# raulmur/ORB_SLAM2

Hardware: NVIDIA H100
Metric: stereo frames/sec (ORB extract L+R + ComputeStereoMatches, KITTI-shaped 1242x375 @2000 kpts) (higher is better)
Workload: dtype u8

## Files before the change

orb_slam2_b200/csrc/k_quadtree.cu:

```cuda
#include "borb_internal.h"

namespace borb {

namespace {

typedef unsigned long long u64;

struct QtView {
    short *bx0[2], *bx1[2], *by0[2], *by1[2];
    int* cnt[2];
    int *cc, *tbl, *order, *scanA, *scanB, *divided, *misc;
    u64* keys;
};

__host__ __device__ inline int pow2_ge(int v) { int k = 1; while (k < v) k <<= 1; return k; }

__device__ inline QtView carve(unsigned char* base, int C, int K) {
    QtView v;
    u64* k = reinterpret_cast<u64*>(base);
    v.keys = k;
    int* ip = reinterpret_cast<int*>(k + K);
    v.cnt[0] = ip; ip += C;
    v.cnt[1] = ip; ip += C;
    v.cc = ip; ip += 4 * C;
    v.tbl = ip; ip += 4 * C;
    v.order = ip; ip += C;
    v.scanA = ip; ip += C;
    v.scanB = ip; ip += C;
    v.divided = ip; ip += C;
    v.misc = ip; ip += 40;
    short* sp = reinterpret_cast<short*>(ip);
    for (int b = 0; b < 2; b++) {
        v.bx0[b] = sp; sp += C;
        v.bx1[b] = sp; sp += C;
        v.by0[b] = sp; sp += C;
        v.by1[b] = sp; sp += C;
    }
    return v;
}

__device__ int block_exscan(int* a, int m, int* wsum) {
    const int T = blockDim.x, tid = threadIdx.x, lane = tid & 31, w = tid >> 5, nw = T >> 5;
    const int per = (m + T - 1) / T;
    const int beg = min(tid * per, m), end = min(beg + per, m);
    int s = 0;
    for (int i = beg; i < end; i++) s += a[i];
    int incl = s;
#pragma unroll
    for (int off = 1; off < 32; off <<= 1) {
        int t = __shfl_up_sync(0xFFFFFFFFu, incl, off);
        if (lane >= off) incl += t;
    }
    if (lane == 31) wsum[w] = incl;
    __syncthreads();
    if (w == 0) {
        int v = lane < nw ? wsum[lane] : 0;
        int inc2 = v;
#pragma unroll
        for (int off = 1; off < 32; off <<= 1) {
            int t = __shfl_up_sync(0xFFFFFFFFu, inc2, off);
            if (lane >= off) inc2 += t;
        }
        wsum[lane] = inc2 - v;
        if (lane == 31) wsum[32] = inc2;
    }
    __syncthreads();
    int base = wsum[w] + incl - s;
    const int total = wsum[32];
    for (int i = beg; i < end; i++) {
        int t = a[i];
        a[i] = base;
        base += t;
    }
    __syncthreads();
    return total;
}

__device__ __forceinline__ int quadrant(int x, int y, int x0, int x1, int y0, int y1) {
    const int mx = x0 + ((x1 - x0 + 1) >> 1);
    const int my = y0 + ((y1 - y0 + 1) >> 1);
    return (x < mx) ? ((y < my) ? 0 : 2) : ((y < my) ? 1 : 3);
}

}

size_t quadtree_smem_bytes(int node_cap) {
    const int C = node_cap, K = pow2_ge(C);
    return (size_t)K * 8 + (size_t)(2 * C + 8 * C + 4 * C) * 4 + 40 * 4 + (size_t)8 * C * 2 + 64;
}

__global__ void __launch_bounds__(256) quadtree_kernel(const __grid_constant__ Geometry g, const uint32_t* __restrict__ cand,
                                                       const int* __restrict__ cand_cnt, int* __restrict__ pnode,
                                                       uint32_t* __restrict__ sel, int* __restrict__ sel_cnt) {
    extern __shared__ __align__(16) unsigned char smem_raw[];
    const int img = blockIdx.y, l = blockIdx.x;
    const LevelGeom& L = g.lv[l];
    const int tid = threadIdx.x, T = blockDim.x;
    const int C = L.node_cap, K = pow2_ge(C);
    QtView v = carve(smem_raw, C, K);
    const int P = min(cand_cnt[img * g.nlevels + l], L.cand_cap);
    const int N = L.quota;
    const uint32_t* pts = cand + (size_t)img * g.cand_image_stride + L.cand_off;
    int* pn = pnode + (size_t)img * g.cand_image_stride + L.cand_off;
    uint32_t* out = sel + (size_t)img * g.sel_image_stride + L.sel_off;
    if (P == 0) {
        if (tid == 0) sel_cnt[img * g.nlevels + l] = 0;
        return;
    }
    const int nIni = L.nIni;
    const float hX = L.hX;
    for (int i = tid; i < nIni; i += T) v.cc[i] = 0;
    __syncthreads();
    for (int p = tid; p < P; p += T) {
        const int x = xys_x(pts[p]) - MIN_BORDER;
        int r = (int)__fdiv_rn((float)x, hX);
        r = min(max(r, 0), nIni - 1);
        atomicAdd(&v.cc[r], 1);
        pn[p] = r;
    }
    __syncthreads();
    for (int i = tid; i < nIni; i += T) v.scanA[i] = v.cc[i] > 0;
    __syncthreads();
    int n = block_exscan(v.scanA, nIni, v.misc);
    int cur = 0;
    for (int i = tid; i < nIni; i += T)
        if (v.cc[i] > 0) {
            const int j = v.scanA[i];
            v.bx0[0][j] = (short)(int)__fmul_rn(hX, (float)i);
            v.bx1[0][j] = (short)(int)__fmul_rn(hX, (float)(i + 1));
            v.by0[0][j] = 0;
            v.by1[0][j] = (short)(L.h - 2 * MIN_BORDER);
            v.cnt[0][j] = v.cc[i];
            v.tbl[i] = j;
        }
    __syncthreads();
    for (int p = tid; p < P; p += T) pn[p] = v.tbl[pn[p]];
    __syncthreads();

    bool phase2 = false, finish = false;
    while (!finish) {
        const int prevSize = n;
        const short *X0 = v.bx0[cur], *X1 = v.bx1[cur], *Y0 = v.by0[cur], *Y1 = v.by1[cur];
        const int* CN = v.cnt[cur];
        for (int j = tid; j < 4 * n; j += T) v.cc[j] = 0;
        __syncthreads();
        for (int p = tid; p < P; p += T) {
            const int k = pn[p];
            if (CN[k] > 1) {
                const uint32_t e = pts[p];
                const int q = quadrant(xys_x(e) - MIN_BORDER, xys_y(e) - MIN_BORDER, X0[k], X1[k], Y0[k], Y1[k]);
                atomicAdd(&v.cc[4 * k + q], 1);
            }
        }
        __syncthreads();
        for (int k = tid; k < n; k += T) v.scanA[k] = CN[k] > 1;
        __syncthreads();
        const int E = block_exscan(v.scanA, n, v.misc);
        int Dn = E;
        if (!phase2) {
            for (int k = tid; k < n; k += T)
                if (CN[k] > 1) v.order[v.scanA[k]] = k;
            __syncthreads();
        } else {
            for (int i = tid; i < K; i += T)
                v.keys[i] = (i < n && CN[i] > 1) ? (((u64)(0xFFFFFFFFu - (unsigned)CN[i]) << 32) | (unsigned)i) : ~0ull;
            __syncthreads();
            for (int kk = 2; kk <= K; kk <<= 1)
                for (int j = kk >> 1; j > 0; j >>= 1) {
                    for (int i = tid; i < K; i += T) {
                        const int ixj = i ^ j;
                        if (ixj > i) {
                            const bool asc = (i & kk) == 0;
                            const u64 a = v.keys[i], b = v.keys[ixj];
                            if ((a > b) == asc) { v.keys[i] = b; v.keys[ixj] = a; }
                        }
                    }
                    __syncthreads();
                }
            for (int r = tid; r < E; r += T) v.order[r] = (int)(v.keys[r] & 0xFFFFFFFFull);
            if (tid == 0) v.misc[33] = E;
            __syncthreads();
            for (int r = tid; r < E; r += T) {
                const int k = v.order[r];
                v.scanA[r] = (v.cc[4 * k] > 0) + (v.cc[4 * k + 1] > 0) + (v.cc[4 * k + 2] > 0) + (v.cc[4 * k + 3] > 0) - 1;
            }
            __syncthreads();
            block_exscan(v.scanA, E, v.misc);
            for (int r = tid; r < E; r += T) {
                const int k = v.order[r];
                const int d = (v.cc[4 * k] > 0) + (v.cc[4 * k + 1] > 0) + (v.cc[4 * k + 2] > 0) + (v.cc[4 * k + 3] > 0) - 1;
                if (n + v.scanA[r] + d >= N) atomicMin(&v.misc[33], r);
            }
            __syncthreads();
            Dn = min(v.misc[33] + 1, E);
            __syncthreads();
        }
        for (int k = tid; k < n; k += T) v.divided[k] = 0;
        __syncthreads();
        for (int r = tid; r < Dn; r += T) v.divided[v.order[r]] = 1;
        for (int r = tid; r < E; r += T) {
            const int k = v.order[r];
            v.scanA[r] = r < Dn ? (v.cc[4 * k] > 0) + (v.cc[4 * k + 1] > 0) + (v.cc[4 * k + 2] > 0) + (v.cc[4 * k + 3] > 0) : 0;
        }
        __syncthreads();
        const int totalCreated = block_exscan(v.scanA, E, v.misc);
        for (int k = tid; k < n; k += T) v.scanB[k] = !v.divided[k];
        __syncthreads();
        const int totalUnd = block_exscan(v.scanB, n, v.misc);
        const int nxt = cur ^ 1;
        if (tid == 0) v.misc[34] = 0;
        __syncthreads();
        int big = 0;
        for (int r = tid; r < Dn; r += T) {
            const int k = v.order[r];
            int c = v.scanA[r];
            const int x0 = X0[k], x1 = X1[k], y0 = Y0[k], y1 = Y1[k];
            const int mx = x0 + ((x1 - x0 + 1) >> 1), my = y0 + ((y1 - y0 + 1) >> 1);
#pragma unroll
            for (int q = 0; q < 4; q++) {
                const int cq = v.cc[4 * k + q];
                if (cq > 0) {
                    const int j = totalCreated - 1 - c;
                    c++;
                    v.tbl[4 * k + q] = j;
                    v.bx0[nxt][j] = (short)((q & 1) ? mx : x0);
                    v.bx1[nxt][j] = (short)((q & 1) ? x1 : mx);
                    v.by0[nxt][j] = (short)((q & 2) ? my : y0);
                    v.by1[nxt][j] = (short)((q & 2) ? y1 : my);
                    v.cnt[nxt][j] = cq;
                    big += cq > 1;
                }
            }
        }
        for (int k = tid; k < n; k += T)
            if (!v.divided[k]) {
                const int j = totalCreated + v.scanB[k];
                v.tbl[4 * k] = j;
                v.bx0[nxt][j] = X0[k]; v.bx1[nxt][j] = X1[k]; v.by0[nxt][j] = Y0[k]; v.by1[nxt][j] = Y1[k];
                v.cnt[nxt][j] = CN[k];
            }
        if (big) atomicAdd(&v.misc[34], big);
        __syncthreads();
        for (int p = tid; p < P; p += T) {
            const int k = pn[p];
            if (v.divided[k]) {
                const uint32_t e = pts[p];
                const int q = quadrant(xys_x(e) - MIN_BORDER, xys_y(e) - MIN_BORDER, X0[k], X1[k], Y0[k], Y1[k]);
                pn[p] = v.tbl[4 * k + q];
            } else
                pn[p] = v.tbl[4 * k];
        }
        const int nToExpand = v.misc[34];
        n = totalCreated + totalUnd;
        cur = nxt;
        __syncthreads();
        if (n >= N || n == prevSize) finish = true;
        else if (!phase2 && n + 3 * nToExpand > N) phase2 = true;
    }
    u64* best = v.keys;
    for (int k = tid; k < n; k += T) best[k] = 0;
    __syncthreads();
    const u64 ORD_MASK = (1ull << 40) - 1;
    for (int p = tid; p < P; p += T) {
        const uint32_t e = pts[p];
        const int x = xys_x(e), y = xys_y(e);
        const u64 ord = ((u64)((y - EDGE) / L.hCell) << 32) | ((u64)((x - EDGE) / L.wCell) << 24) | ((u64)y << 12) | (u64)x;
        const u64 key = ((u64)xys_s(e) << 40) | (ORD_MASK - ord);
        atomicMax(&best[pn[p]], key);
    }
    __syncthreads();
    for (int k = tid; k < n; k += T) {
        const u64 key = best[k];
        const u64 ord = ORD_MASK - (key & ORD_MASK);
        out[k] = pack_xys((int)(ord & 0xFFF), (int)((ord >> 12) & 0xFFF), (int)(key >> 40));
    }
    if (tid == 0) sel_cnt[img * g.nlevels + l] = n;
}

int launch_quadtree(const Geometry& g, const Workspace& ws, int n_images, cudaStream_t s) {
    int maxC = 0;
    for (int l = 0; l < g.nlevels; l++) maxC = g.lv[l].node_cap > maxC ? g.lv[l].node_cap : maxC;
    const size_t smem = quadtree_smem_bytes(maxC);
    allow_max_smem((const void*)quadtree_kernel);
    dim3 grid(g.nlevels, n_images);
    quadtree_kernel<<<grid, 256, smem, s>>>(g, ws.cand, ws.cand_cnt, ws.pnode, ws.sel, ws.sel_cnt);
    return 1;
}

}
```

Before: 37720.

## Restructure quadtree kernel: register-resident points, fused scans, rank-based ordering

Rewrites the ORB quadtree distribution kernel. Candidate points and their node ids are held in registers when the count fits (up to 20 per thread), so per-iteration global reads and writes of pnode are avoided. Node boxes are packed as short4. Divide and keep are fused into a single scan callback with a packed 16/16-bit counter, and the next level's vote is done right after the move, removing several passes and barriers. The phase-2 bitonic sort is replaced with an O(n^2) rank count, which is cheaper for small node counts but scales poorly if nodes grow, and the extra registers may cost occupancy.

```diff
diff --git a/orb_slam2_b200/csrc/k_quadtree.cu b/orb_slam2_b200/csrc/k_quadtree.cu
--- a/orb_slam2_b200/csrc/k_quadtree.cu
+++ b/orb_slam2_b200/csrc/k_quadtree.cu
@@ -4,47 +4,47 @@
 
 namespace {
 
-typedef unsigned long long u64;
+constexpr int QT_THREADS = 256;
+constexpr int QT_PPT = 20;
+constexpr int QT_ONCHIP = QT_THREADS * QT_PPT;
 
 struct QtView {
-    short *bx0[2], *bx1[2], *by0[2], *by1[2];
+    int* cc[2];
+    short4* box[2];
     int* cnt[2];
-    int *cc, *tbl, *order, *scanA, *scanB, *divided, *misc;
-    u64* keys;
+    int* tbl;
+    int* order;
+    int* rank;
+    int* pre;
+    int* misc;
 };
 
-__host__ __device__ inline int pow2_ge(int v) { int k = 1; while (k < v) k <<= 1; return k; }
-
-__device__ inline QtView carve(unsigned char* base, int C, int K) {
+__device__ inline QtView carve(unsigned char* base, int C) {
     QtView v;
-    u64* k = reinterpret_cast<u64*>(base);
-    v.keys = k;
-    int* ip = reinterpret_cast<int*>(k + K);
+    int* ip = reinterpret_cast<int*>(base);
+    v.cc[0] = ip; ip += 4 * C;
+    v.cc[1] = ip; ip += 4 * C;
+    short4* bp = reinterpret_cast<short4*>(ip);
+    v.box[0] = bp; bp += C;
+    v.box[1] = bp; bp += C;
+    ip = reinterpret_cast<int*>(bp);
     v.cnt[0] = ip; ip += C;
     v.cnt[1] = ip; ip += C;
-    v.cc = ip; ip += 4 * C;
     v.tbl = ip; ip += 4 * C;
     v.order = ip; ip += C;
-    v.scanA = ip; ip += C;
-    v.scanB = ip; ip += C;
-    v.divided = ip; ip += C;
-    v.misc = ip; ip += 40;
-    short* sp = reinterpret_cast<short*>(ip);
-    for (int b = 0; b < 2; b++) {
-        v.bx0[b] = sp; sp += C;
-        v.bx1[b] = sp; sp += C;
-        v.by0[b] = sp; sp += C;
-        v.by1[b] = sp; sp += C;
-    }
+    v.rank = ip; ip += C;
+    v.pre = ip; ip += C + 1;
+    v.misc = ip;
     return v;
 }
 
-__device__ int block_exscan(int* a, int m, int* wsum) {
-    const int T = blockDim.x, tid = threadIdx.x, lane = tid & 31, w = tid >> 5, nw = T >> 5;
-    const int per = (m + T - 1) / T;
+template <class V, class U>
+__device__ __forceinline__ int block_exscan(int m, int* wsum, V val, U use) {
+    const int tid = threadIdx.x, lane = tid & 31, w = tid >> 5, nw = QT_THREADS >> 5;
+    const int per = (m + QT_THREADS - 1) / QT_THREADS;
     const int beg = min(tid * per, m), end = min(beg + per, m);
     int s = 0;
-    for (int i = beg; i < end; i++) s += a[i];
+    for (int i = beg; i < end; i++) s += val(i);
     int incl = s;
 #pragma unroll
     for (int off = 1; off < 32; off <<= 1) {
@@ -54,50 +54,70 @@
     if (lane == 31) wsum[w] = incl;
     __syncthreads();
     if (w == 0) {
-        int v = lane < nw ? wsum[lane] : 0;
-        int inc2 = v;
+        int x = lane < nw ? wsum[lane] : 0;
+        int inc2 = x;
 #pragma unroll
         for (int off = 1; off < 32; off <<= 1) {
             int t = __shfl_up_sync(0xFFFFFFFFu, inc2, off);
             if (lane >= off) inc2 += t;
         }
-        wsum[lane] = inc2 - v;
+        wsum[lane] = inc2 - x;
         if (lane == 31) wsum[32] = inc2;
     }
     __syncthreads();
     int base = wsum[w] + incl - s;
     const int total = wsum[32];
     for (int i = beg; i < end; i++) {
-        int t = a[i];
-        a[i] = base;
+        const int t = val(i);
+        use(i, base, total);
         base += t;
     }
-    __syncthreads();
     return total;
 }
 
-__device__ __forceinline__ int quadrant(int x, int y, int x0, int x1, int y0, int y1) {
-    const int mx = x0 + ((x1 - x0 + 1) >> 1);
-    const int my = y0 + ((y1 - y0 + 1) >> 1);
+__device__ __forceinline__ int quadrant(uint32_t e, short4 b) {
+    const int x = xys_x(e) - MIN_BORDER, y = xys_y(e) - MIN_BORDER;
+    const int mx = b.x + ((b.y - b.x + 1) >> 1);
+    const int my = b.z + ((b.w - b.z + 1) >> 1);
     return (x < mx) ? ((y < my) ? 0 : 2) : ((y < my) ? 1 : 3);
 }
 
+template <bool READ, bool WRITE, class F>
+__device__ __forceinline__ void for_points(bool onchip, int P, const uint32_t (&e)[QT_PPT], uint32_t (&nd)[QT_PPT / 2],
+                                           const uint32_t* __restrict__ pts, int* __restrict__ pn, F f) {
+    if (onchip) {
+#pragma unroll
+        for (int i = 0; i < QT_PPT; i++)
+            if (threadIdx.x + i * QT_THREADS < P) {
+                const int sh = 16 * (i & 1);
+                int s = (nd[i / 2] >> sh) & 0xFFFF;
+                f(e[i], s);
+                if (WRITE) nd[i / 2] = (nd[i / 2] & ~(0xFFFFu << sh)) | ((uint32_t)s << sh);
+            }
+    } else {
+        for (int p = threadIdx.x; p < P; p += QT_THREADS) {
+            int s = READ ? pn[p] : 0;
+            f(pts[p], s);
+            if (WRITE) pn[p] = s;
+        }
+    }
+}
+
 }
 
 size_t quadtree_smem_bytes(int node_cap) {
-    const int C = node_cap, K = pow2_ge(C);
-    return (size_t)K * 8 + (size_t)(2 * C + 8 * C + 4 * C) * 4 + 40 * 4 + (size_t)8 * C * 2 + 64;
-}
-
-__global__ void __launch_bounds__(256) quadtree_kernel(const __grid_constant__ Geometry g, const uint32_t* __restrict__ cand,
-                                                       const int* __restrict__ cand_cnt, int* __restrict__ pnode,
-                                                       uint32_t* __restrict__ sel, int* __restrict__ sel_cnt) {
+    const size_t C = (size_t)node_cap;
+    return C * (2 * 4 * 4 + 2 * 8 + 2 * 4 + 4 * 4 + 3 * 4) + 4 + 35 * 4;
+}
+
+__global__ void __launch_bounds__(QT_THREADS, 4) quadtree_kernel(const __grid_constant__ Geometry g, const uint32_t* __restrict__ cand,
+                                                                 const int* __restrict__ cand_cnt, int* __restrict__ pnode,
+                                                                 uint32_t* __restrict__ sel, int* __restrict__ sel_cnt) {
     extern __shared__ __align__(16) unsigned char smem_raw[];
     const int img = blockIdx.y, l = blockIdx.x;
     const LevelGeom& L = g.lv[l];
-    const int tid = threadIdx.x, T = blockDim.x;
-    const int C = L.node_cap, K = pow2_ge(C);
-    QtView v = carve(smem_raw, C, K);
+    const int tid = threadIdx.x, T = QT_THREADS;
+    QtView v = carve(smem_raw, L.node_cap);
     const int P = min(cand_cnt[img * g.nlevels + l], L.cand_cap);
     const int N = L.quota;
     const uint32_t* pts = cand + (size_t)img * g.cand_image_stride + L.cand_off;
@@ -107,174 +127,141 @@
         if (tid == 0) sel_cnt[img * g.nlevels + l] = 0;
         return;
     }
+    const bool onchip = P <= QT_ONCHIP;
+    uint32_t e[QT_PPT], nd[QT_PPT / 2] = {};
+    if (onchip) {
+#pragma unroll
+        for (int i = 0; i < QT_PPT; i++) e[i] = tid + i * T < P ? pts[tid + i * T] : 0u;
+    }
     const int nIni = L.nIni;
     const float hX = L.hX;
-    for (int i = tid; i < nIni; i += T) v.cc[i] = 0;
-    __syncthreads();
-    for (int p = tid; p < P; p += T) {
-        const int x = xys_x(pts[p]) - MIN_BORDER;
-        int r = (int)__fdiv_rn((float)x, hX);
-        r = min(max(r, 0), nIni - 1);
-        atomicAdd(&v.cc[r], 1);
-        pn[p] = r;
-    }
-    __syncthreads();
-    for (int i = tid; i < nIni; i += T) v.scanA[i] = v.cc[i] > 0;
-    __syncthreads();
-    int n = block_exscan(v.scanA, nIni, v.misc);
-    int cur = 0;
-    for (int i = tid; i < nIni; i += T)
-        if (v.cc[i] > 0) {
-            const int j = v.scanA[i];
-            v.bx0[0][j] = (short)(int)__fmul_rn(hX, (float)i);
-            v.bx1[0][j] = (short)(int)__fmul_rn(hX, (float)(i + 1));
-            v.by0[0][j] = 0;
-            v.by1[0][j] = (short)(L.h - 2 * MIN_BORDER);
-            v.cnt[0][j] = v.cc[i];
+    int* rc = v.cc[1];
+    for (int i = tid; i < nIni; i += T) rc[i] = 0;
+    __syncthreads();
+    for_points<false, true>(onchip, P, e, nd, pts, pn, [&](uint32_t x, int& s) {
+        const int r = (int)__fdiv_rn((float)(xys_x(x) - MIN_BORDER), hX);
+        s = min(max(r, 0), nIni - 1);
+        atomicAdd(&rc[s], 1);
+    });
+    __syncthreads();
+    int n = block_exscan(nIni, v.misc, [&](int i) { return rc[i] > 0; }, [&](int i, int j, int) {
+        if (rc[i] > 0) {
+            v.box[0][j] = make_short4((short)(int)__fmul_rn(hX, (float)i), (short)(int)__fmul_rn(hX, (float)(i + 1)), 0,
+                                      (short)(L.h - 2 * MIN_BORDER));
+            v.cnt[0][j] = rc[i];
             v.tbl[i] = j;
         }
-    __syncthreads();
-    for (int p = tid; p < P; p += T) pn[p] = v.tbl[pn[p]];
-    __syncthreads();
-
-    bool phase2 = false, finish = false;
-    while (!finish) {
-        const int prevSize = n;
-        const short *X0 = v.bx0[cur], *X1 = v.bx1[cur], *Y0 = v.by0[cur], *Y1 = v.by1[cur];
-        const int* CN = v.cnt[cur];
-        for (int j = tid; j < 4 * n; j += T) v.cc[j] = 0;
-        __syncthreads();
-        for (int p = tid; p < P; p += T) {
-            const int k = pn[p];
-            if (CN[k] > 1) {
-                const uint32_t e = pts[p];
-                const int q = quadrant(xys_x(e) - MIN_BORDER, xys_y(e) - MIN_BORDER, X0[k], X1[k], Y0[k], Y1[k]);
-                atomicAdd(&v.cc[4 * k + q], 1);
-            }
-        }
-        __syncthreads();
-        for (int k = tid; k < n; k += T) v.scanA[k] = CN[k] > 1;
-        __syncthreads();
-        const int E = block_exscan(v.scanA, n, v.misc);
-        int Dn = E;
-        if (!phase2) {
-            for (int k = tid; k < n; k += T)
-                if (CN[k] > 1) v.order[v.scanA[k]] = k;
-            __syncthreads();
-        } else {
-            for (int i = tid; i < K; i += T)
-                v.keys[i] = (i < n && CN[i] > 1) ? (((u64)(0xFFFFFFFFu - (unsigned)CN[i]) << 32) | (unsigned)i) : ~0ull;
-            __syncthreads();
-            for (int kk = 2; kk <= K; kk <<= 1)
-                for (int j = kk >> 1; j > 0; j >>= 1) {
-                    for (int i = tid; i < K; i += T) {
-                        const int ixj = i ^ j;
-                        if (ixj > i) {
-                            const bool asc = (i & kk) == 0;
-                            const u64 a = v.keys[i], b = v.keys[ixj];
-                            if ((a > b) == asc) { v.keys[i] = b; v.keys[ixj] = a; }
-                        }
-                    }
-                    __syncthreads();
-                }
-            for (int r = tid; r < E; r += T) v.order[r] = (int)(v.keys[r] & 0xFFFFFFFFull);
-            if (tid == 0) v.misc[33] = E;
-            __syncthreads();
-            for (int r = tid; r < E; r += T) {
-                const int k = v.order[r];
-                v.scanA[r] = (v.cc[4 * k] > 0) + (v.cc[4 * k + 1] > 0) + (v.cc[4 * k + 2] > 0) + (v.cc[4 * k + 3] > 0) - 1;
-            }
-            __syncthreads();
-            block_exscan(v.scanA, E, v.misc);
-            for (int r = tid; r < E; r += T) {
-                const int k = v.order[r];
-                const int d = (v.cc[4 * k] > 0) + (v.cc[4 * k + 1] > 0) + (v.cc[4 * k + 2] > 0) + (v.cc[4 * k + 3] > 0) - 1;
-                if (n + v.scanA[r] + d >= N) atomicMin(&v.misc[33], r);
-            }
-            __syncthreads();
-            Dn = min(v.misc[33] + 1, E);
-            __syncthreads();
-        }
-        for (int k = tid; k < n; k += T) v.divided[k] = 0;
-        __syncthreads();
-        for (int r = tid; r < Dn; r += T) v.divided[v.order[r]] = 1;
-        for (int r = tid; r < E; r += T) {
-            const int k = v.order[r];
-            v.scanA[r] = r < Dn ? (v.cc[4 * k] > 0) + (v.cc[4 * k + 1] > 0) + (v.cc[4 * k + 2] > 0) + (v.cc[4 * k + 3] > 0) : 0;
-        }
-        __syncthreads();
-        const int totalCreated = block_exscan(v.scanA, E, v.misc);
-        for (int k = tid; k < n; k += T) v.scanB[k] = !v.divided[k];
-        __syncthreads();
-        const int totalUnd = block_exscan(v.scanB, n, v.misc);
-        const int nxt = cur ^ 1;
-        if (tid == 0) v.misc[34] = 0;
-        __syncthreads();
+    });
+    for (int j = n + tid; j < ((n + 3) & ~3); j += T) v.cnt[0][j] = 0;
+    for (int j = tid; j < 4 * n; j += T) v.cc[0][j] = 0;
+    __syncthreads();
+    short4 *B = v.box[0], *NB = v.box[1];
+    int *CN = v.cnt[0], *NCN = v.cnt[1], *CC = v.cc[0], *NCC = v.cc[1];
+    auto move_and_vote = [&](const short4* bx, int* cc) {
+        for_points<true, true>(onchip, P, e, nd, pts, pn, [&](uint32_t x, int& s) {
+            const int k = v.tbl[s];
+            s = 4 * k + quadrant(x, bx[k]);
+        });
+        for_points<true, false>(onchip, P, e, nd, pts, pn, [&](uint32_t, int& s) { atomicAdd(&cc[s], 1); });
+    };
+    move_and_vote(B, CC);
+    __syncthreads();
+
+    int E = 0, nn;
+    bool phase2 = false;
+    for (;;) {
+        auto children = [&](int k) { return (CC[4 * k] > 0) + (CC[4 * k + 1] > 0) + (CC[4 * k + 2] > 0) + (CC[4 * k + 3] > 0); };
         int big = 0;
-        for (int r = tid; r < Dn; r += T) {
-            const int k = v.order[r];
-            int c = v.scanA[r];
-            const int x0 = X0[k], x1 = X1[k], y0 = Y0[k], y1 = Y1[k];
-            const int mx = x0 + ((x1 - x0 + 1) >> 1), my = y0 + ((y1 - y0 + 1) >> 1);
+        auto divide = [&](int k, int j) {
+            const short4 b = B[k];
+            const short mx = (short)(b.x + ((b.y - b.x + 1) >> 1)), my = (short)(b.z + ((b.w - b.z + 1) >> 1));
 #pragma unroll
             for (int q = 0; q < 4; q++) {
-                const int cq = v.cc[4 * k + q];
+                const int cq = CC[4 * k + q];
                 if (cq > 0) {
-                    const int j = totalCreated - 1 - c;
-                    c++;
                     v.tbl[4 * k + q] = j;
-                    v.bx0[nxt][j] = (short)((q & 1) ? mx : x0);
-                    v.bx1[nxt][j] = (short)((q & 1) ? x1 : mx);
-                    v.by0[nxt][j] = (short)((q & 2) ? my : y0);
-                    v.by1[nxt][j] = (short)((q & 2) ? y1 : my);
-                    v.cnt[nxt][j] = cq;
+                    NB[j] = make_short4((q & 1) ? mx : b.x, (q & 1) ? b.y : mx, (q & 2) ? my : b.z, (q & 2) ? b.w : my);
+                    NCN[j] = cq;
                     big += cq > 1;
+                    j--;
                 }
             }
-        }
-        for (int k = tid; k < n; k += T)
-            if (!v.divided[k]) {
-                const int j = totalCreated + v.scanB[k];
-                v.tbl[4 * k] = j;
-                v.bx0[nxt][j] = X0[k]; v.bx1[nxt][j] = X1[k]; v.by0[nxt][j] = Y0[k]; v.by1[nxt][j] = Y1[k];
-                v.cnt[nxt][j] = CN[k];
+        };
+        auto keep = [&](int k, int j) {
+            v.tbl[4 * k] = v.tbl[4 * k + 1] = v.tbl[4 * k + 2] = v.tbl[4 * k + 3] = j;
+            NB[j] = B[k];
+            NCN[j] = CN[k];
+        };
+        if (tid == 0) v.misc[34] = 0;
+        int created;
+        if (!phase2) {
+            const int tot = block_exscan(n, v.misc, [&](int k) { return CN[k] > 1 ? children(k) << 16 : 1; }, [&](int k, int pre, int total) {
+                if (CN[k] > 1) divide(k, (total >> 16) - 1 - (pre >> 16));
+                else keep(k, (total >> 16) + (pre & 0xFFFF));
+            });
+            created = tot >> 16;
+            nn = created + (tot & 0xFFFF);
+        } else {
+            const int4* CN4 = reinterpret_cast<const int4*>(CN);
+            for (int k = tid; k < n; k += T) {
+                const int s = CN[k];
+                if (s > 1) {
+                    int r = 0;
+                    for (int j = 0; j < n; j += 4) {
+                        const int4 c = CN4[j >> 2];
+                        r += (c.x + (j < k) > s) + (c.y + (j + 1 < k) > s) + (c.z + (j + 2 < k) > s) + (c.w + (j + 3 < k) > s);
+                    }
+                    v.order[r] = k;
+                    v.rank[k] = r;
+                } else
+                    v.rank[k] = E;
             }
+            if (tid == 0) { v.misc[33] = E; v.pre[0] = 0; }
+            __syncthreads();
+            block_exscan(E, v.misc, [&](int r) { return children(v.order[r]) - 1; }, [&](int r, int pre, int) {
+                const int d = children(v.order[r]) - 1;
+                v.pre[r + 1] = pre + d;
+                if (n + pre + d >= N) atomicMin(&v.misc[33], r);
+            });
+            __syncthreads();
+            const int Dn = min(v.misc[33] + 1, E);
+            created = v.pre[Dn] + Dn;
+            for (int r = tid; r < Dn; r += T) divide(v.order[r], created - 1 - v.pre[r] - r);
+            nn = created + block_exscan(n, v.misc, [&](int k) { return v.rank[k] >= Dn; }, [&](int k, int pre, int) {
+                if (v.rank[k] >= Dn) keep(k, created + pre);
+            });
+        }
         if (big) atomicAdd(&v.misc[34], big);
+        const bool last = nn >= N || nn == n;
+        for (int j = tid; j < 4 * nn; j += T) NCC[j] = 0;
+        for (int j = nn + tid; j < ((nn + 3) & ~3); j += T) NCN[j] = 0;
         __syncthreads();
-        for (int p = tid; p < P; p += T) {
-            const int k = pn[p];
-            if (v.divided[k]) {
-                const uint32_t e = pts[p];
-                const int q = quadrant(xys_x(e) - MIN_BORDER, xys_y(e) - MIN_BORDER, X0[k], X1[k], Y0[k], Y1[k]);
-                pn[p] = v.tbl[4 * k + q];
-            } else
-                pn[p] = v.tbl[4 * k];
-        }
+        if (last) break;
         const int nToExpand = v.misc[34];
-        n = totalCreated + totalUnd;
-        cur = nxt;
+        move_and_vote(NB, NCC);
         __syncthreads();
-        if (n >= N || n == prevSize) finish = true;
-        else if (!phase2 && n + 3 * nToExpand > N) phase2 = true;
-    }
-    u64* best = v.keys;
-    for (int k = tid; k < n; k += T) best[k] = 0;
-    __syncthreads();
+        if (!phase2 && nn + 3 * nToExpand > N) phase2 = true;
+        n = nn;
+        E = nToExpand;
+        short4* tb = B; B = NB; NB = tb;
+        int* tc = CN; CN = NCN; NCN = tc;
+        tc = CC; CC = NCC; NCC = tc;
+    }
+    typedef unsigned long long u64;
     const u64 ORD_MASK = (1ull << 40) - 1;
-    for (int p = tid; p < P; p += T) {
-        const uint32_t e = pts[p];
-        const int x = xys_x(e), y = xys_y(e);
-        const u64 ord = ((u64)((y - EDGE) / L.hCell) << 32) | ((u64)((x - EDGE) / L.wCell) << 24) | ((u64)y << 12) | (u64)x;
-        const u64 key = ((u64)xys_s(e) << 40) | (ORD_MASK - ord);
-        atomicMax(&best[pn[p]], key);
-    }
-    __syncthreads();
-    for (int k = tid; k < n; k += T) {
+    u64* best = reinterpret_cast<u64*>(NCC);
+    for_points<true, false>(onchip, P, e, nd, pts, pn, [&](uint32_t x, int& s) {
+        const int xx = xys_x(x), yy = xys_y(x);
+        const u64 ord = ((u64)((yy - EDGE) / L.hCell) << 32) | ((u64)((xx - EDGE) / L.wCell) << 24) | ((u64)yy << 12) | (u64)xx;
+        atomicMax(&best[v.tbl[s]], ((u64)xys_s(x) << 40) | (ORD_MASK - ord));
+    });
+    __syncthreads();
+    for (int k = tid; k < nn; k += T) {
         const u64 key = best[k];
         const u64 ord = ORD_MASK - (key & ORD_MASK);
         out[k] = pack_xys((int)(ord & 0xFFF), (int)((ord >> 12) & 0xFFF), (int)(key >> 40));
     }
-    if (tid == 0) sel_cnt[img * g.nlevels + l] = n;
+    if (tid == 0) sel_cnt[img * g.nlevels + l] = nn;
 }
 
 int launch_quadtree(const Geometry& g, const Workspace& ws, int n_images, cudaStream_t s) {
@@ -283,7 +270,7 @@
     const size_t smem = quadtree_smem_bytes(maxC);
     allow_max_smem((const void*)quadtree_kernel);
     dim3 grid(g.nlevels, n_images);
-    quadtree_kernel<<<grid, 256, smem, s>>>(g, ws.cand, ws.cand_cnt, ws.pnode, ws.sel, ws.sel_cnt);
+    quadtree_kernel<<<grid, QT_THREADS, smem, s>>>(g, ws.cand, ws.cand_cnt, ws.pnode, ws.sel, ws.sel_cnt);
     return 1;
 }
 
```

New measurement: 39610 (median of 6 runs). 5.0% higher.
